# taishan1994/pytorch-distributed-NLP

Measured on NVIDIA H100. Metric: training samples/sec (seq_len=128), higher is better.
Workload: dtype bf16

## Files before the change

pytorch-distributed-nlp_b200/csrc/common.cuh:

```cuda
#pragma once
#include <cuda.h>
#include <cuda_bf16.h>
#include <cuda_runtime.h>
#include <stdint.h>
#include <cstdio>
#include "wgmma.cuh"

namespace b2 {

void set_error(const char* fmt, ...);
int32_t check_cuda(cudaError_t e, const char* what);
void count_launches(int n);
#define B2_CUDA(expr)                                                   \
  do {                                                                  \
    int32_t _s = ::b2::check_cuda((expr), #expr);                       \
    if (_s != 0) return _s;                                             \
  } while (0)
#define B2_REQUIRE(cond, ...)                                           \
  do {                                                                  \
    if (!(cond)) {                                                      \
      ::b2::set_error(__VA_ARGS__);                                     \
      return -2;                                                        \
    }                                                                   \
  } while (0)

int32_t get_tensor_map_2d(CUtensorMap* out, const void* base, uint64_t rows, uint64_t cols,
                          uint64_t pitch_bytes, uint32_t box_rows, uint32_t box_cols);

#ifdef __CUDACC__
template <typename... KArgs, typename... Args>
inline void launch_kernel(void (*kernel)(KArgs...), dim3 grid, dim3 block, size_t smem, cudaStream_t stream,
                          Args&&... args) {
  cudaLaunchConfig_t cfg = {};
  cfg.gridDim = grid;
  cfg.blockDim = block;
  cfg.dynamicSmemBytes = smem;
  cfg.stream = stream;
  cudaLaunchAttribute attr[1];
  attr[0].id = cudaLaunchAttributeProgrammaticStreamSerialization;
  attr[0].val.programmaticStreamSerializationAllowed = 1;
  cfg.attrs = attr;
  cfg.numAttrs = 1;
  (void)cudaLaunchKernelEx(&cfg, kernel, static_cast<KArgs>(args)...);
}
#define B2_LAUNCH(kernel, grid, block, smem, stream, ...) \
  ::b2::launch_kernel(kernel, dim3(grid), dim3(block), (size_t)(smem), (cudaStream_t)(stream), ##__VA_ARGS__)

__device__ __forceinline__ uint32_t smem_u32(const void* p) {
  return static_cast<uint32_t>(__cvta_generic_to_shared(p));
}
__device__ __forceinline__ uint8_t* smem_align_1024(uint8_t* smem_raw) {
  return smem_raw + ((1024u - (smem_u32(smem_raw) & 1023u)) & 1023u);
}
__device__ __forceinline__ uint32_t lane_id() { return threadIdx.x & 31; }

__device__ __forceinline__ float warp_sum(float v) {
#pragma unroll
  for (int o = 16; o > 0; o >>= 1) v += __shfl_xor_sync(0xffffffffu, v, o);
  return v;
}
__device__ __forceinline__ float warp_max(float v) {
#pragma unroll
  for (int o = 16; o > 0; o >>= 1) v = fmaxf(v, __shfl_xor_sync(0xffffffffu, v, o));
  return v;
}

__device__ __forceinline__ uint32_t pack_bf16(float lo, float hi) {
  __nv_bfloat162 t = __floats2bfloat162_rn(lo, hi);
  return *reinterpret_cast<uint32_t*>(&t);
}
__device__ __forceinline__ float bf16_lo(uint32_t v) { return __uint_as_float(v << 16); }
__device__ __forceinline__ float bf16_hi(uint32_t v) { return __uint_as_float(v & 0xffff0000u); }
__device__ __forceinline__ float bf16_round(float x) {
  return __bfloat162float(__float2bfloat16_rn(x));
}

__device__ __forceinline__ void gelu_hq(float x, float& hq, float& e) {
  float t;
  asm("ex2.approx.ftz.f32 %0, %1;" : "=f"(e) : "f"((x * x) * -0.72134752044448170f));
  asm("rcp.approx.ftz.f32 %0, %1;" : "=f"(t) : "f"(fmaf(fabsf(x), 0.23164189f, 1.0f)));
  float poly = fmaf(0.5307027145f, t, -0.7265760135f);
  poly = fmaf(poly, t, 0.7107068705f);
  poly = fmaf(poly, t, -0.142248368f);
  poly = fmaf(poly, t, 0.127414796f);
  hq = (poly * t) * e;
}
__device__ __forceinline__ float gelu_erf(float x) {
  float hq, e;
  gelu_hq(x, hq, e);
  return fmaf(-fabsf(x), hq, fmaxf(x, 0.f));
}
__device__ __forceinline__ float gelu_erf_grad(float x) {
  float hq, e;
  gelu_hq(x, hq, e);
  const float cdf = x >= 0.f ? 1.0f - hq : hq;
  return fmaf(x * 0.3989422804014327f, e, cdf);
}
__device__ __forceinline__ float ex2_approx(float x) {
  float y;
  asm("ex2.approx.ftz.f32 %0, %1;" : "=f"(y) : "f"(x));
  return y;
}
__device__ __forceinline__ uint32_t pack_bf16_round(float& lo, float& hi) {
  const uint32_t u = pack_bf16(lo, hi);
  lo = bf16_lo(u);
  hi = bf16_hi(u);
  return u;
}

struct Philox4 {
  uint32_t x, y, z, w;
};
__device__ __forceinline__ Philox4 philox4x32_10(uint32_t c0, uint32_t c1, uint32_t c2, uint32_t c3,
                                                 uint32_t k0, uint32_t k1) {
  const uint32_t M0 = 0xD2511F53u, M1 = 0xCD9E8D57u, W0 = 0x9E3779B9u, W1 = 0xBB67AE85u;
#pragma unroll
  for (int r = 0; r < 10; ++r) {
    const uint32_t hi0 = __umulhi(M0, c0), lo0 = M0 * c0;
    const uint32_t hi1 = __umulhi(M1, c2), lo1 = M1 * c2;
    const uint32_t n0 = hi1 ^ c1 ^ k0, n1 = lo1, n2 = hi0 ^ c3 ^ k1, n3 = lo0;
    c0 = n0; c1 = n1; c2 = n2; c3 = n3;
    k0 += W0; k1 += W1;
  }
  return Philox4{c0, c1, c2, c3};
}

struct DropCtx {
  uint32_t k0, k1, step, site, thresh;
  float scale;
};
__device__ __forceinline__ DropCtx make_drop_ctx(const unsigned long long* rng, uint32_t site, float p) {
  DropCtx d;
  unsigned long long seed = rng ? rng[0] : 0ull;
  unsigned long long step = rng ? rng[1] : 0ull;
  d.k0 = (uint32_t)seed; d.k1 = (uint32_t)(seed >> 32);
  d.step = (uint32_t)step; d.site = site;
  d.thresh = (uint32_t)(p * 65536.0f + 0.5f);
  d.scale = (p > 0.f) ? 1.0f / (1.0f - p) : 1.0f;
  return d;
}
__device__ __forceinline__ uint32_t dropout_keep8(const DropCtx& d, unsigned long long idx) {
  if (d.thresh == 0) return 0xffu;
  const unsigned long long g = idx >> 3;
  Philox4 r = philox4x32_10((uint32_t)g, (uint32_t)(g >> 32), d.site, d.step, d.k0, d.k1);
  uint32_t m = 0;
  m |= ((r.x & 0xffffu) >= d.thresh) << 0;
  m |= ((r.x >> 16) >= d.thresh) << 1;
  m |= ((r.y & 0xffffu) >= d.thresh) << 2;
  m |= ((r.y >> 16) >= d.thresh) << 3;
  m |= ((r.z & 0xffffu) >= d.thresh) << 4;
  m |= ((r.z >> 16) >= d.thresh) << 5;
  m |= ((r.w & 0xffffu) >= d.thresh) << 6;
  m |= ((r.w >> 16) >= d.thresh) << 7;
  return m;
}

__device__ __forceinline__ void mbar_init(uint64_t* bar, uint32_t count) {
  asm volatile("mbarrier.init.shared::cta.b64 [%0], %1;" ::"r"(smem_u32(bar)), "r"(count) : "memory");
}
__device__ __forceinline__ void fence_mbar_init() {
  asm volatile("fence.mbarrier_init.release.cluster;" ::: "memory");
}
__device__ __forceinline__ void mbar_expect_tx(uint64_t* bar, uint32_t bytes) {
  asm volatile("mbarrier.arrive.expect_tx.shared::cta.b64 _, [%0], %1;" ::"r"(smem_u32(bar)), "r"(bytes)
               : "memory");
}
__device__ __forceinline__ void mbar_arrive(uint64_t* bar) {
  asm volatile("mbarrier.arrive.shared::cta.b64 _, [%0];" ::"r"(smem_u32(bar)) : "memory");
}
__device__ __forceinline__ bool mbar_try_wait(uint64_t* bar, uint32_t parity) {
  uint32_t ok;
  asm volatile(
      "{\n\t.reg .pred p;\n\t"
      "mbarrier.try_wait.parity.shared::cta.b64 p, [%1], %2;\n\t"
      "selp.u32 %0, 1, 0, p;\n\t}"
      : "=r"(ok)
      : "r"(smem_u32(bar)), "r"(parity)
      : "memory");
  return ok != 0;
}
__device__ __forceinline__ void mbar_wait(uint64_t* bar, uint32_t parity) {
  uint32_t spins = 0;
  while (!mbar_try_wait(bar, parity)) {
    if (++spins > (1u << 24)) __trap();
  }
}

__device__ __forceinline__ void fence_proxy_async_smem() {
  asm volatile("fence.proxy.async.shared::cta;" ::: "memory");
}

__device__ __forceinline__ void tma_prefetch_desc(const CUtensorMap* m) {
  asm volatile("prefetch.tensormap [%0];" ::"l"(reinterpret_cast<uint64_t>(m)) : "memory");
}
__device__ __forceinline__ void tma_load_2d(void* smem_dst, const CUtensorMap* m, uint64_t* bar, int32_t c0,
                                            int32_t c1) {
  asm volatile(
      "cp.async.bulk.tensor.2d.shared::cluster.global.mbarrier::complete_tx::bytes [%0], [%1, {%3, %4}], [%2];"
      ::"r"(smem_u32(smem_dst)),
      "l"(reinterpret_cast<uint64_t>(m)), "r"(smem_u32(bar)), "r"(c0), "r"(c1)
      : "memory");
}
__device__ __forceinline__ void tma_store_2d(const CUtensorMap* m, const void* smem_src, int32_t c0, int32_t c1) {
  asm volatile("cp.async.bulk.tensor.2d.global.shared::cta.bulk_group [%0, {%2, %3}], [%1];" ::"l"(
                   reinterpret_cast<uint64_t>(m)),
               "r"(smem_u32(smem_src)), "r"(c0), "r"(c1)
               : "memory");
}
__device__ __forceinline__ void tma_store_commit_and_wait() {
  asm volatile("cp.async.bulk.commit_group;" ::: "memory");
  asm volatile("cp.async.bulk.wait_group 0;" ::: "memory");
}

__device__ __forceinline__ uint32_t cluster_ctarank() {
  uint32_t r;
  asm volatile("mov.u32 %0, %%cluster_ctarank;" : "=r"(r));
  return r;
}
__device__ __forceinline__ uint32_t mapa_u32(uint32_t smem_addr, uint32_t rank) {
  uint32_t r;
  asm volatile("mapa.shared::cluster.u32 %0, %1, %2;" : "=r"(r) : "r"(smem_addr), "r"(rank));
  return r;
}
__device__ __forceinline__ void st_cluster_f32x2(uint32_t cluster_addr, float a, float b) {
  asm volatile("st.shared::cluster.v2.f32 [%0], {%1, %2};" ::"r"(cluster_addr), "f"(a), "f"(b) : "memory");
}
__device__ __forceinline__ void cluster_sync_all() {
  asm volatile("barrier.cluster.arrive.release.aligned;\n\tbarrier.cluster.wait.acquire.aligned;" ::: "memory");
}
__device__ __forceinline__ void named_barrier_sync(uint32_t id, uint32_t count) {
  asm volatile("bar.sync %0, %1;" ::"r"(id), "r"(count) : "memory");
}

__device__ __forceinline__ uint64_t make_smem_desc(uint32_t saddr, uint32_t lbo_bytes, uint32_t sbo_bytes) {
  uint64_t d = 0;
  d |= (uint64_t)((saddr >> 4) & 0x3fffu);
  d |= (uint64_t)((lbo_bytes >> 4) & 0x3fffu) << 16;
  d |= (uint64_t)((sbo_bytes >> 4) & 0x3fffu) << 32;
  d |= (uint64_t)1 << 62;
  return d;
}

__device__ __forceinline__ void pdl_wait() { asm volatile("griddepcontrol.wait;" ::: "memory"); }
__device__ __forceinline__ void pdl_launch_dependents() { asm volatile("griddepcontrol.launch_dependents;" ::: "memory"); }

__device__ __forceinline__ uint4 ldg16(const void* p) { return __ldg(reinterpret_cast<const uint4*>(p)); }
__device__ __forceinline__ void stg16(void* p, uint4 v) { *reinterpret_cast<uint4*>(p) = v; }
#endif

}
```

pytorch-distributed-nlp_b200/csrc/gemm.cu:

```cuda
#include "common.cuh"
#include "gemm_epilogue.cuh"
#include "../../include/b2_ddp_bert.h"

namespace b2 {

constexpr int BM = 128;
constexpr int BK = 64;
constexpr int WGMMA_K = 16;
constexpr int kGemmThreads = (4 + kEpiWarps) * 32;

template <int BN>
struct GemmCfg {
  static constexpr int kABytes = BM * BK * 2;
  static constexpr int kBBytes = BN * BK * 2;
  static constexpr int kStageBytes = kABytes + kBBytes;
  static constexpr int kStages = (BN == 256) ? 4 : 6;
  static constexpr int kPipeBytes = kStages * kStageBytes;
  static constexpr int kAccLd = BN + 4;
  static constexpr int kSmemBytes = kPipeBytes + kEpiWarps * kEpiStageBytes + 1024  + 256 ;
  static_assert(BM * kAccLd * 4 <= kPipeBytes, "the accumulator tile lives in the drained operand ring");
};

template <int BN, bool A_MN, bool B_MN>
__device__ __forceinline__ void gemm_mainloop(uint8_t* smem, uint64_t* full_bar, uint64_t* empty_bar,
                                              const CUtensorMap* tmap_a, const CUtensorMap* tmap_b, int m0, int n0,
                                              int kb0, int kb1, int warp, int lane) {
  using Cfg = GemmCfg<BN>;
  if (warp == 0) {
    if (lane == 0) {
      int stage = 0; uint32_t phase = 0;
      for (int kb = kb0; kb < kb1; ++kb) {
        mbar_wait(&empty_bar[stage], phase ^ 1);
        mbar_expect_tx(&full_bar[stage], Cfg::kStageBytes);
        uint8_t* sa = smem + stage * Cfg::kStageBytes;
        uint8_t* sb = sa + Cfg::kABytes;
        const int k0 = kb * BK;
        if (!A_MN) {
          tma_load_2d(sa, tmap_a, &full_bar[stage], k0, m0);
        } else {
#pragma unroll
          for (int j = 0; j < BM / 64; ++j)
            tma_load_2d(sa + j * (BK * 128), tmap_a, &full_bar[stage], m0 + 64 * j, k0);
        }
        if (!B_MN) {
          tma_load_2d(sb, tmap_b, &full_bar[stage], k0, n0);
        } else {
#pragma unroll
          for (int j = 0; j < BN / 64; ++j)
            tma_load_2d(sb + j * (BK * 128), tmap_b, &full_bar[stage], n0 + 64 * j, k0);
        }
        if (++stage == Cfg::kStages) { stage = 0; phase ^= 1; }
      }
    }
  } else if (warp >= 4) {
    const int wg = (warp - 4) >> 2;
    constexpr uint32_t a_lbo = A_MN ? BK * 128 : 16, b_lbo = B_MN ? BK * 128 : 16;
    constexpr uint32_t a_kstep = A_MN ? WGMMA_K * 128 : WGMMA_K * 2;
    constexpr uint32_t b_kstep = B_MN ? WGMMA_K * 128 : WGMMA_K * 2;
    float acc[BN / 2];
#pragma unroll
    for (int i = 0; i < BN / 2; ++i) acc[i] = 0.f;
    int stage = 0, prev = -1; uint32_t phase = 0;
    for (int kb = kb0; kb < kb1; ++kb) {
      mbar_wait(&full_bar[stage], phase);
      const uint32_t sa = smem_u32(smem + stage * Cfg::kStageBytes) + wg * 8192;
      const uint32_t sb = smem_u32(smem + stage * Cfg::kStageBytes + Cfg::kABytes);
      wgmma_fence();
#pragma unroll
      for (int k = 0; k < BK / WGMMA_K; ++k)
        wgmma_bf16<BN, A_MN ? 1 : 0, B_MN ? 1 : 0>(acc, make_smem_desc(sa + k * a_kstep, a_lbo, 1024),
                                                     make_smem_desc(sb + k * b_kstep, b_lbo, 1024),
                                                     (kb > kb0 || k > 0) ? 1u : 0u);
      wgmma_commit();
      wgmma_wait<1>();
      if (prev >= 0 && lane == 0) mbar_arrive(&empty_bar[prev]);
      prev = stage;
      if (++stage == Cfg::kStages) { stage = 0; phase ^= 1; }
    }
    wgmma_wait<0>();
    wgmma_fence_regs(acc);
    if (prev >= 0 && lane == 0) mbar_arrive(&empty_bar[prev]);
    named_barrier_sync(1, kEpiWarps * 32);
    float* accs = reinterpret_cast<float*>(smem);
    const int r = wg * 64 + (warp & 3) * 16 + (lane >> 2);
    const int c = 2 * (lane & 3);
#pragma unroll
    for (int j = 0; j < BN / 8; ++j) {
      *reinterpret_cast<float2*>(accs + (size_t)r * Cfg::kAccLd + 8 * j + c) = make_float2(acc[4 * j], acc[4 * j + 1]);
      *reinterpret_cast<float2*>(accs + (size_t)(r + 8) * Cfg::kAccLd + 8 * j + c) =
          make_float2(acc[4 * j + 2], acc[4 * j + 3]);
    }
    named_barrier_sync(1, kEpiWarps * 32);
  }
}

template <int BN>
__device__ __forceinline__ void gemm_setup(uint64_t* full_bar, uint64_t* empty_bar) {
  if (threadIdx.x == 0) {
    for (int s = 0; s < GemmCfg<BN>::kStages; ++s) {
      mbar_init(&full_bar[s], 1);
      mbar_init(&empty_bar[s], kEpiWarps);
    }
    fence_mbar_init();
  }
  __syncthreads();
}

template <int BN, bool A_MN, bool B_MN>
__global__ void __launch_bounds__(kGemmThreads, 1)
gemm_bf16_kernel(const __grid_constant__ CUtensorMap tmap_a, const __grid_constant__ CUtensorMap tmap_b,
                 const GemmKernelParams p) {
  using Cfg = GemmCfg<BN>;
  extern __shared__ uint8_t smem_raw[];
  uint8_t* smem = smem_align_1024(smem_raw);
  uint8_t* epi_stage = smem + Cfg::kPipeBytes;
  uint64_t* full_bar = reinterpret_cast<uint64_t*>(epi_stage + kEpiWarps * kEpiStageBytes);
  uint64_t* empty_bar = full_bar + Cfg::kStages;
  const int warp = threadIdx.x >> 5;
  const int lane = threadIdx.x & 31;
  if (threadIdx.x == 0) {
    tma_prefetch_desc(&tmap_a);
    tma_prefetch_desc(&tmap_b);
  }
  gemm_setup<BN>(full_bar, empty_bar);
  pdl_wait();
  pdl_launch_dependents();

  const int tile = blockIdx.x / p.splits, split = blockIdx.x % p.splits;
  const int m0 = (tile / p.tiles_n) * BM, n0 = (tile % p.tiles_n) * BN;
  const int kb0 = split * p.kblocks_per_split;
  const int kb1 = min(kb0 + p.kblocks_per_split, p.kblocks_total);
  gemm_mainloop<BN, A_MN, B_MN>(smem, full_bar, empty_bar, &tmap_a, &tmap_b, m0, n0, kb0, kb1, warp, lane);
  if (warp >= 4) {
    const DropCtx drop = make_drop_ctx(p.rng, p.rng_site, p.dropout_p);
    epilogue_tile<BN>(p, drop, reinterpret_cast<const float*>(smem), Cfg::kAccLd, warp, lane, m0, n0, split,
                      epi_stage + (warp - 4) * kEpiStageBytes);
  }
}

constexpr int kMaxGroup = 4;
struct GroupedProblem {
  int M, N, tiles_n, tile_begin;
  __nv_bfloat16* D; long long ldd;
};
struct GroupedParams {
  int count, num_work, kblocks;
  GroupedProblem pr[kMaxGroup];
};

struct GroupedMaps {
  CUtensorMap a[kMaxGroup], b[kMaxGroup];
};
__device__ __forceinline__ int grouped_find(const GroupedParams& gp, int w) {
  int pi = 0;
#pragma unroll
  for (int i = 1; i < kMaxGroup; ++i)
    if (i < gp.count && w >= gp.pr[i].tile_begin) pi = i;
  return pi;
}

__global__ void __launch_bounds__(kGemmThreads, 1)
gemm_grouped_tn_kernel(const __grid_constant__ GroupedMaps maps, const GroupedParams gp) {
  constexpr int BN = 256;
  using Cfg = GemmCfg<BN>;
  extern __shared__ uint8_t smem_raw[];
  uint8_t* smem = smem_align_1024(smem_raw);
  uint8_t* epi_stage = smem + Cfg::kPipeBytes;
  uint64_t* full_bar = reinterpret_cast<uint64_t*>(epi_stage + kEpiWarps * kEpiStageBytes);
  uint64_t* empty_bar = full_bar + Cfg::kStages;
  const int warp = threadIdx.x >> 5;
  const int lane = threadIdx.x & 31;
  const int pi = grouped_find(gp, blockIdx.x);
  if (threadIdx.x == 0) {
    tma_prefetch_desc(&maps.a[pi]);
    tma_prefetch_desc(&maps.b[pi]);
  }
  gemm_setup<BN>(full_bar, empty_bar);
  pdl_wait();
  pdl_launch_dependents();

  const GroupedProblem& pr = gp.pr[pi];
  const int lt = blockIdx.x - pr.tile_begin;
  const int m0 = (lt / pr.tiles_n) * BM;
  const int n0 = (lt % pr.tiles_n) * BN;
  gemm_mainloop<BN, true, true>(smem, full_bar, empty_bar, &maps.a[pi], &maps.b[pi], m0, n0, 0, gp.kblocks, warp,
                                lane);
  if (warp < 4) return;
  uint8_t* stage = epi_stage + (warp - 4) * kEpiStageBytes;
  GemmKernelParams q;
  q.splits = 1; q.epilogue = B2_EPI_NONE; q.bias = nullptr; q.aux_in = nullptr; q.aux_out = nullptr;
  q.partial = nullptr; q.dropout_p = 0.f; q.rng = nullptr; q.rng_site = 0; q.timing = nullptr; q.colsum = nullptr;
  q.ld_aux_in = 0; q.ld_aux_out = 0; q.K = 0; q.tiles_m = 0; q.kblocks_per_split = 0; q.kblocks_total = 0;
  q.M = pr.M; q.N = pr.N; q.tiles_n = pr.tiles_n; q.D = pr.D; q.ldd = pr.ldd;
  DropCtx drop;
  drop.k0 = 0; drop.k1 = 0; drop.step = 0; drop.site = 0; drop.thresh = 0; drop.scale = 1.f;
  epilogue_tile<BN>(q, drop, reinterpret_cast<const float*>(smem), Cfg::kAccLd, warp, lane, m0, n0, 0, stage);
}

__global__ void splitk_reduce_kernel(const float* __restrict__ partial, __nv_bfloat16* __restrict__ D,
                                     long long ldd, int M, int N, int splits) {
  pdl_wait();
  pdl_launch_dependents();
  const long long idx = (long long)blockIdx.x * blockDim.x + threadIdx.x;
  const long long total = (long long)M * N / 4;
  if (idx >= total) return;
  const long long e = idx * 4;
  const int m = (int)(e / N), n = (int)(e % N);
  float4 acc = make_float4(0.f, 0.f, 0.f, 0.f);
  for (int s = 0; s < splits; ++s) {
    const float4 v = *reinterpret_cast<const float4*>(partial + (size_t)s * M * N + e);
    acc.x += v.x; acc.y += v.y; acc.z += v.z; acc.w += v.w;
  }
  uint2 o;
  o.x = pack_bf16(acc.x, acc.y);
  o.y = pack_bf16(acc.z, acc.w);
  *reinterpret_cast<uint2*>(D + (size_t)m * ldd + n) = o;
}

static int g_num_sms = 0;
static int num_sms() {
  if (g_num_sms == 0) {
    int dev = 0;
    cudaGetDevice(&dev);
    cudaDeviceGetAttribute(&g_num_sms, cudaDevAttrMultiProcessorCount, dev);
    if (g_num_sms <= 0) g_num_sms = 132;
  }
  return g_num_sms;
}

static void fill_params(GemmKernelParams& p, const b2_gemm_args_t& a, int tile_m, int bn, int splits) {
  p.M = (int)a.M; p.N = (int)a.N; p.K = (int)a.K;
  p.tiles_m = (p.M + tile_m - 1) / tile_m;
  p.tiles_n = (p.N + bn - 1) / bn;
  p.kblocks_total = (p.K + BK - 1) / BK;
  p.splits = splits;
  p.kblocks_per_split = (p.kblocks_total + splits - 1) / splits;
  p.epilogue = (splits > 1 && a.epilogue != B2_EPI_ACCUM_F32) ? B2_EPI_PARTIAL_F32 : a.epilogue;
  p.D = (__nv_bfloat16*)a.D; p.ldd = a.ldd;
  p.bias = (const __nv_bfloat16*)a.bias;
  p.aux_in = (const __nv_bfloat16*)a.aux_in; p.ld_aux_in = a.ld_aux_in;
  p.aux_out = (__nv_bfloat16*)a.aux_out; p.ld_aux_out = a.ld_aux_out;
  p.partial = (float*)a.workspace;
  p.dropout_p = a.dropout_p; p.rng = (const unsigned long long*)a.rng_state; p.rng_site = a.rng_site;
  p.timing = (long long*)a.debug_timing;
  p.colsum = a.colsum_out;
}

static int32_t launch_splitk_reduce(const b2_gemm_args_t& a, int splits, cudaStream_t stream) {
  const long long total = (long long)a.M * a.N / 4;
  B2_LAUNCH(splitk_reduce_kernel, (unsigned)((total + 255) / 256), 256, 0, stream, 
      (const float*)a.workspace, (__nv_bfloat16*)a.D, a.ldd, (int)a.M, (int)a.N, splits);
  B2_CUDA(cudaGetLastError());
  count_launches(1);
  return 0;
}

template <int BN, bool A_MN, bool B_MN>
static int32_t launch_gemm(const b2_gemm_args_t& a, int splits, cudaStream_t stream) {
  using Cfg = GemmCfg<BN>;
  CUtensorMap ta, tb;
  int32_t st;
  if (!A_MN) st = get_tensor_map_2d(&ta, a.A, (uint64_t)a.M, (uint64_t)a.K, (uint64_t)a.lda * 2, BM, 64);
  else       st = get_tensor_map_2d(&ta, a.A, (uint64_t)a.K, (uint64_t)a.M, (uint64_t)a.lda * 2, BK, 64);
  if (st) return st;
  if (!B_MN) st = get_tensor_map_2d(&tb, a.B, (uint64_t)a.N, (uint64_t)a.K, (uint64_t)a.ldb * 2, BN, 64);
  else       st = get_tensor_map_2d(&tb, a.B, (uint64_t)a.K, (uint64_t)a.N, (uint64_t)a.ldb * 2, BK, 64);
  if (st) return st;
  GemmKernelParams p;
  fill_params(p, a, BM, BN, splits);
  auto kern = gemm_bf16_kernel<BN, A_MN, B_MN>;
  static bool attr_set = false;
  if (!attr_set) {
    B2_CUDA(cudaFuncSetAttribute(kern, cudaFuncAttributeMaxDynamicSharedMemorySize, Cfg::kSmemBytes));
    attr_set = true;
  }
  const int work = p.tiles_m * p.tiles_n * p.splits;
  B2_LAUNCH(kern, work, kGemmThreads, Cfg::kSmemBytes, stream, ta, tb, p);
  B2_CUDA(cudaGetLastError());
  count_launches(1);
  if (splits > 1 && a.epilogue != B2_EPI_ACCUM_F32) return launch_splitk_reduce(a, splits, stream);
  return 0;
}

struct Choice { int bn, splits; };
static Choice choose_config(const b2_gemm_args_t& a) {
  const int sms = num_sms();
  const int kblocks = (int)((a.K + BK - 1) / BK);
  const bool accum = a.epilogue == B2_EPI_ACCUM_F32;
  const bool can_split = accum || ((a.epilogue == B2_EPI_NONE) && a.workspace != nullptr && a.bias == nullptr);
  double best = 1e30;
  Choice c{128, 1};
  const double l2_bytes_per_cycle = 3000.0;
  const int bns[2] = {256, 128};
  for (int bi = 0; bi < 2; ++bi) {
    const int bn = bns[bi];
    if (a.N % bn != 0 && bn != 128) continue;
    const int tiles = (int)((a.M + BM - 1) / BM) * (int)((a.N + bn - 1) / bn);
    const int max_s = can_split ? 8 : 1;
    for (int s = 1; s <= max_s; s = accum ? s + 1 : s * 2) {
      if (s > 1 && (kblocks / s < 8)) break;
      if (s > 1 && !accum && (size_t)s * a.M * a.N * 4 > (size_t)a.workspace_bytes) break;
      const int work = tiles * s;
      const int rounds = (work + sms - 1) / sms;
      const int busy_sms = work < sms ? work : sms;
      const double mma_cycles = 128.0 * bn * 64 / 2048.0;
      const double bytes_per_sm = (128 + bn) * 128.0;
      const double feed_cycles = bytes_per_sm * busy_sms / l2_bytes_per_cycle;
      const double kb_cycles = mma_cycles > feed_cycles ? mma_cycles : feed_cycles;
      double t = rounds * ((double)((kblocks + s - 1) / s) * kb_cycles + 2500.0 );
      if (s > 1 && !accum) t += 1500.0 + (double)s * a.M * a.N * 8 / 3000.0;
      if (s > 1 && accum) t += (double)(s - 1) * a.M * a.N * 4 / 3000.0;
      if (t < best) { best = t; c = Choice{bn, s}; }
    }
  }
  return c;
}

}

using namespace b2;

extern "C" int32_t b2_gemm_bf16(const b2_gemm_args_t* a, void* stream_) {
  cudaStream_t stream = (cudaStream_t)stream_;
  B2_REQUIRE(a != nullptr, "b2_gemm_bf16: null args");
  B2_REQUIRE(a->M > 0 && a->N > 0 && a->K > 0, "b2_gemm_bf16: empty problem M=%lld N=%lld K=%lld",
             (long long)a->M, (long long)a->N, (long long)a->K);
  B2_REQUIRE(a->A && a->B && a->D, "b2_gemm_bf16: null operand pointer");
  B2_REQUIRE(a->N % 64 == 0, "b2_gemm_bf16: N=%lld must be a multiple of 64", (long long)a->N);
  B2_REQUIRE(a->K % 8 == 0 && a->lda % 8 == 0 && a->ldb % 8 == 0 && a->ldd % 8 == 0,
             "b2_gemm_bf16: K and leading dimensions must be multiples of 8 elements (16 B)");
  B2_REQUIRE(((uintptr_t)a->A % 16 == 0) && ((uintptr_t)a->B % 16 == 0) && ((uintptr_t)a->D % 16 == 0),
             "b2_gemm_bf16: operands must be 16-byte aligned");
  B2_REQUIRE(a->epilogue >= B2_EPI_NONE && a->epilogue <= B2_EPI_ACCUM_F32, "b2_gemm_bf16: bad epilogue %d",
             a->epilogue);
  if (a->epilogue == B2_EPI_BIAS || a->epilogue == B2_EPI_BIAS_GELU || a->epilogue == B2_EPI_BIAS_DROPOUT_RESIDUAL)
    B2_REQUIRE(a->bias != nullptr, "b2_gemm_bf16: epilogue %d needs a bias", a->epilogue);
  if (a->epilogue == B2_EPI_BIAS_DROPOUT_RESIDUAL || a->epilogue == B2_EPI_RESIDUAL ||
      a->epilogue == B2_EPI_GELU_BWD || a->epilogue == B2_EPI_RESIDUAL_F32)
    B2_REQUIRE(a->aux_in != nullptr && a->ld_aux_in % 8 == 0, "b2_gemm_bf16: epilogue %d needs aux_in",
               a->epilogue);
  if (a->epilogue == B2_EPI_BIAS_GELU)
    B2_REQUIRE(a->aux_out != nullptr && a->ld_aux_out % 8 == 0, "b2_gemm_bf16: BIAS_GELU needs aux_out");
  if (a->epilogue == B2_EPI_BIAS_DROPOUT_RESIDUAL && a->dropout_p > 0.f)
    B2_REQUIRE(a->rng_state != nullptr, "b2_gemm_bf16: dropout needs rng_state");
  B2_REQUIRE(a->dropout_p >= 0.f && a->dropout_p < 1.f, "b2_gemm_bf16: dropout_p out of range");

  Choice c = choose_config(*a);
  if (a->force_bn == 128 || a->force_bn == 256) {
    B2_REQUIRE(a->N % a->force_bn == 0 || a->force_bn == 128, "b2_gemm_bf16: force_bn does not divide N");
    c.bn = a->force_bn;
  }
  if (a->force_splits >= 1) {
    B2_REQUIRE(a->force_splits == 1 ||
                   a->epilogue == B2_EPI_ACCUM_F32 ||
                   (a->epilogue == B2_EPI_NONE && a->workspace &&
                    (size_t)a->force_splits * a->M * a->N * 4 <= (size_t)a->workspace_bytes),
               "b2_gemm_bf16: split-K needs EPI_ACCUM_F32, or EPI_NONE and a large enough workspace");
    c.splits = a->force_splits;
  }
  const bool a_mn = a->a_major == B2_MAJOR_MN, b_mn = a->b_major == B2_MAJOR_MN;
  B2_REQUIRE(!(a_mn && !b_mn), "b2_gemm_bf16: layout TT (A MN-major, B K-major) is not on the path");

#define B2_DISPATCH(BN_)                                                          \
  if (c.bn == BN_) {                                                              \
    if (!a_mn && !b_mn) return launch_gemm<BN_, false, false>(*a, c.splits, stream); \
    if (!a_mn && b_mn) return launch_gemm<BN_, false, true>(*a, c.splits, stream);   \
    return launch_gemm<BN_, true, true>(*a, c.splits, stream);                       \
  }
  B2_DISPATCH(128)
  B2_DISPATCH(256)
#undef B2_DISPATCH
  set_error("b2_gemm_bf16: no kernel for BN=%d", c.bn);
  return -2;
}

extern "C" int32_t b2_gemm_bf16_grouped(const b2_gemm_args_t* args, int32_t count, void* stream_) {
  cudaStream_t stream = (cudaStream_t)stream_;
  B2_REQUIRE(args != nullptr && count >= 1, "b2_gemm_bf16_grouped: no problems");
  bool groupable = count <= kMaxGroup;
  for (int i = 0; i < count && groupable; ++i) {
    const b2_gemm_args_t& a = args[i];
    groupable = a.a_major == B2_MAJOR_MN && a.b_major == B2_MAJOR_MN && a.epilogue == B2_EPI_NONE &&
                a.bias == nullptr && a.colsum_out == nullptr && a.N % 256 == 0 && a.K == args[0].K && a.M > 0 &&
                a.K > 0 && a.A && a.B && a.D && a.K % 8 == 0 && a.lda % 8 == 0 && a.ldb % 8 == 0 &&
                a.ldd % 8 == 0 && ((uintptr_t)a.A % 16 == 0) && ((uintptr_t)a.B % 16 == 0) &&
                ((uintptr_t)a.D % 16 == 0) && a.force_splits <= 1 &&
                (a.force_bn == 0 || a.force_bn == 256);
  }
  if (!groupable) {
    for (int i = 0; i < count; ++i) {
      const int32_t st = b2_gemm_bf16(&args[i], stream_);
      if (st) return st;
    }
    return 0;
  }
  GroupedMaps maps;
  GroupedParams gp;
  gp.count = count;
  gp.kblocks = (int)((args[0].K + BK - 1) / BK);
  int work = 0;
  for (int i = 0; i < count; ++i) {
    const b2_gemm_args_t& a = args[i];
    int32_t st = get_tensor_map_2d(&maps.a[i], a.A, (uint64_t)a.K, (uint64_t)a.M, (uint64_t)a.lda * 2, BK, 64);
    if (st) return st;
    st = get_tensor_map_2d(&maps.b[i], a.B, (uint64_t)a.K, (uint64_t)a.N, (uint64_t)a.ldb * 2, BK, 64);
    if (st) return st;
    GroupedProblem& g = gp.pr[i];
    g.M = (int)a.M; g.N = (int)a.N; g.tiles_n = (int)(a.N / 256); g.tile_begin = work;
    g.D = (__nv_bfloat16*)a.D; g.ldd = a.ldd;
    work += (int)((a.M + BM - 1) / BM) * g.tiles_n;
  }
  for (int i = count; i < kMaxGroup; ++i) { gp.pr[i] = gp.pr[0]; gp.pr[i].tile_begin = 0x7fffffff; maps.a[i] = maps.a[0]; maps.b[i] = maps.b[0]; }
  gp.num_work = work;
  static bool attr_set = false;
  if (!attr_set) {
    B2_CUDA(cudaFuncSetAttribute(gemm_grouped_tn_kernel, cudaFuncAttributeMaxDynamicSharedMemorySize,
                                 GemmCfg<256>::kSmemBytes));
    attr_set = true;
  }
  B2_LAUNCH(gemm_grouped_tn_kernel, work, kGemmThreads, GemmCfg<256>::kSmemBytes, stream, maps, gp);
  B2_CUDA(cudaGetLastError());
  count_launches(1);
  return 0;
}
```

pytorch-distributed-nlp_b200/csrc/gemm_epilogue.cuh:

```cuda
#pragma once
#include "common.cuh"
#include "../../include/b2_ddp_bert.h"

namespace b2 {

struct GemmKernelParams {
  int M, N, K;
  int tiles_m, tiles_n, splits, kblocks_per_split, kblocks_total;
  int epilogue;
  __nv_bfloat16* D; long long ldd;
  const __nv_bfloat16* bias;
  const __nv_bfloat16* aux_in; long long ld_aux_in;
  __nv_bfloat16* aux_out; long long ld_aux_out;
  float* partial;
  float dropout_p; const unsigned long long* rng; unsigned rng_site;
  long long* timing;
  float* colsum;
};

constexpr int kEpiStageBytes = 32 * 128;

#ifdef __CUDACC__
template <int CH>
__device__ __forceinline__ uint4* stage_ptr(uint8_t* stage, int row, int chunk) {
  if (CH == 8) return reinterpret_cast<uint4*>(stage + row * 128 + ((chunk ^ (row & 7)) << 4));
  return reinterpret_cast<uint4*>(stage + (row >> 1) * 128 + (((((row & 1) << 2) | chunk) ^ ((row >> 1) & 7)) << 4));
}
template <int CH>
__device__ __forceinline__ void tile_s2g(uint8_t* stage, uint8_t* g, long long pitch, int lane, int rows_valid) {
  constexpr int RPS = 32 / CH;
#pragma unroll
  for (int k = 0; k < CH; ++k) {
    const int r = RPS * k + lane / CH, c = lane % CH;
    const uint4 v = *stage_ptr<CH>(stage, r, c);
    if (r < rows_valid) *reinterpret_cast<uint4*>(g + (size_t)r * pitch + c * 16) = v;
  }
}
__device__ __forceinline__ void tile_s2g_red_f32(uint8_t* stage, uint8_t* g, long long pitch, int lane,
                                                 int rows_valid) {
#pragma unroll
  for (int k = 0; k < 8; ++k) {
    const int r = 4 * k + (lane >> 3), c = lane & 7;
    const uint4 v = *stage_ptr<8>(stage, r, c);
    if (r < rows_valid)
      asm volatile("red.global.add.v4.f32 [%0], {%1, %2, %3, %4};" ::"l"(g + (size_t)r * pitch + c * 16),
                   "f"(__uint_as_float(v.x)), "f"(__uint_as_float(v.y)), "f"(__uint_as_float(v.z)),
                   "f"(__uint_as_float(v.w))
                   : "memory");
  }
}
template <int CH>
__device__ __forceinline__ void tile_g2s_async(uint8_t* stage, const uint8_t* g, long long pitch, int lane,
                                               int rows_valid) {
  constexpr int RPS = 32 / CH;
#pragma unroll
  for (int k = 0; k < CH; ++k) {
    const int r = RPS * k + lane / CH, c = lane % CH;
    uint4* dst = stage_ptr<CH>(stage, r, c);
    if (r < rows_valid) {
      asm volatile("cp.async.cg.shared.global [%0], [%1], 16;" ::"r"(smem_u32(dst)), "l"(g + (size_t)r * pitch + c * 16)
                   : "memory");
    } else {
      *dst = make_uint4(0u, 0u, 0u, 0u);
    }
  }
  asm volatile("cp.async.commit_group;" ::: "memory");
}
__device__ __forceinline__ void tile_async_wait() { asm volatile("cp.async.wait_group 0;" ::: "memory"); }

__device__ __forceinline__ void acc_ld32(const float* a, uint32_t (&v)[32]) {
#pragma unroll
  for (int k = 0; k < 8; ++k) {
    const uint4 t = *reinterpret_cast<const uint4*>(a + 4 * k);
    v[4 * k] = t.x; v[4 * k + 1] = t.y; v[4 * k + 2] = t.z; v[4 * k + 3] = t.w;
  }
}

template <int CH>
__device__ __forceinline__ void row_write32(uint8_t* stage, int lane, int c0, const float (&f)[32]) {
#pragma unroll
  for (int c = 0; c < 4; ++c) {
    uint4 o;
    o.x = pack_bf16(f[8 * c + 0], f[8 * c + 1]); o.y = pack_bf16(f[8 * c + 2], f[8 * c + 3]);
    o.z = pack_bf16(f[8 * c + 4], f[8 * c + 5]); o.w = pack_bf16(f[8 * c + 6], f[8 * c + 7]);
    *stage_ptr<CH>(stage, lane, c0 + c) = o;
  }
}
template <int CH>
__device__ __forceinline__ void row_read32(uint8_t* stage, int lane, int c0, float (&r)[32]) {
#pragma unroll
  for (int c = 0; c < 4; ++c) {
    const uint4 t = *stage_ptr<CH>(stage, lane, c0 + c);
    r[8 * c + 0] = bf16_lo(t.x); r[8 * c + 1] = bf16_hi(t.x); r[8 * c + 2] = bf16_lo(t.y); r[8 * c + 3] = bf16_hi(t.y);
    r[8 * c + 4] = bf16_lo(t.z); r[8 * c + 5] = bf16_hi(t.z); r[8 * c + 6] = bf16_lo(t.w); r[8 * c + 7] = bf16_hi(t.w);
  }
}

constexpr int kEpiWarps = 8;
template <int BN>
__device__ __forceinline__ void epilogue_tile(const GemmKernelParams& p, const DropCtx& drop, const float* acc,
                                              int acc_ld, int warp, int lane, int m_base, int n0, int split,
                                              uint8_t* stage) {
  static_assert(BN == 128 || BN == 256, "tile widths on the path");
  constexpr int kColsPerWarp = BN / 2;
  constexpr int WT = 64;
  constexpr int CH = WT / 8;
  const int quarter = warp & 3;
  const int cgrp = (warp - 4) >> 2;
  const int row0 = m_base + quarter * 32;
  const int rows_valid = p.M - row0;
  const int m = row0 + lane;
  const int nw = n0 + cgrp * kColsPerWarp;
  const float* arow = acc + (size_t)(quarter * 32 + lane) * acc_ld + cgrp * kColsPerWarp;

  if (p.epilogue == B2_EPI_PARTIAL_F32 || p.epilogue == B2_EPI_RESIDUAL_F32 || p.epilogue == B2_EPI_ACCUM_F32) {
    const bool accum = p.epilogue == B2_EPI_ACCUM_F32;
    const bool no_aux = p.epilogue != B2_EPI_RESIDUAL_F32;
    const bool to_ws = p.epilogue == B2_EPI_PARTIAL_F32;
    float* dst_base = to_ws ? p.partial + (size_t)split * p.M * p.N : reinterpret_cast<float*>(p.D);
    const long long dst_ld = to_ws ? (long long)p.N : p.ldd;
    auto prefetch = [&](int c) {
      const int n = nw + c * 32;
      if (!no_aux && n < p.N && rows_valid > 0)
        tile_g2s_async<8>(stage, reinterpret_cast<const uint8_t*>(reinterpret_cast<const float*>(p.aux_in) +
                                                                 (size_t)row0 * p.ld_aux_in + n),
                          p.ld_aux_in * 4, lane, rows_valid);
    };
    prefetch(0);
#pragma unroll 1
    for (int c = 0; c < kColsPerWarp / 32; ++c) {
      const int n = nw + c * 32;
      uint32_t v[32];
      acc_ld32(arow + c * 32, v);
      if (n < p.N && rows_valid > 0) {
        if (!no_aux) {
          if (c > 0) prefetch(c);
          tile_async_wait();
          __syncwarp();
#pragma unroll
          for (int k = 0; k < 8; ++k) {
            const uint4 t = *stage_ptr<8>(stage, lane, k);
            v[4 * k + 0] = __float_as_uint(__uint_as_float(v[4 * k + 0]) + __uint_as_float(t.x));
            v[4 * k + 1] = __float_as_uint(__uint_as_float(v[4 * k + 1]) + __uint_as_float(t.y));
            v[4 * k + 2] = __float_as_uint(__uint_as_float(v[4 * k + 2]) + __uint_as_float(t.z));
            v[4 * k + 3] = __float_as_uint(__uint_as_float(v[4 * k + 3]) + __uint_as_float(t.w));
          }
          __syncwarp();
        }
#pragma unroll
        for (int k = 0; k < 8; ++k)
          *stage_ptr<8>(stage, lane, k) = make_uint4(v[4 * k], v[4 * k + 1], v[4 * k + 2], v[4 * k + 3]);
        __syncwarp();
        uint8_t* gdst = reinterpret_cast<uint8_t*>(dst_base + (size_t)row0 * dst_ld + n);
        if (accum) tile_s2g_red_f32(stage, gdst, dst_ld * 4, lane, rows_valid);
        else       tile_s2g<8>(stage, gdst, dst_ld * 4, lane, rows_valid);
      }
      __syncwarp();
    }
    return;
  }

  const bool has_aux = p.epilogue == B2_EPI_BIAS_DROPOUT_RESIDUAL || p.epilogue == B2_EPI_RESIDUAL ||
                       p.epilogue == B2_EPI_GELU_BWD;
  auto prefetch = [&](int t) {
    const int n = nw + t * WT;
    if (has_aux && n < p.N && rows_valid > 0)
      tile_g2s_async<CH>(stage, reinterpret_cast<const uint8_t*>(p.aux_in + (size_t)row0 * p.ld_aux_in + n),
                         p.ld_aux_in * 2, lane, rows_valid);
  };
  prefetch(0);
#pragma unroll 1
  for (int t = 0; t < kColsPerWarp / WT; ++t) {
    const int n = nw + t * WT;
    const bool active = n < p.N && rows_valid > 0;
    if (has_aux && active) {
      if (t > 0) prefetch(t);
      tile_async_wait();
      __syncwarp();
    }
#pragma unroll 1
    for (int h = 0; h < WT / 32; ++h) {
      float f[32];
      {
        uint32_t v[32];
        acc_ld32(arow + t * WT + h * 32, v);
#pragma unroll
        for (int j = 0; j < 32; ++j) f[j] = __uint_as_float(v[j]);
      }
      if (!active) continue;
      const int nh = n + h * 32;
      if (p.bias != nullptr) {
#pragma unroll
        for (int j = 0; j < 32; j += 8) {
          const uint4 b = ldg16(p.bias + nh + j);
          f[j + 0] += bf16_lo(b.x); f[j + 1] += bf16_hi(b.x); f[j + 2] += bf16_lo(b.y); f[j + 3] += bf16_hi(b.y);
          f[j + 4] += bf16_lo(b.z); f[j + 5] += bf16_hi(b.z); f[j + 6] += bf16_lo(b.w); f[j + 7] += bf16_hi(b.w);
        }
      }
      if (has_aux) {
        float r[32];
        row_read32<CH>(stage, lane, 4 * h, r);
        if (p.epilogue == B2_EPI_BIAS_DROPOUT_RESIDUAL) {
#pragma unroll
          for (int j = 0; j < 32; j += 8) {
            const uint32_t keep = dropout_keep8(drop, (unsigned long long)m * p.N + nh + j);
#pragma unroll
            for (int i = 0; i < 8; ++i) f[j + i] = (((keep >> i) & 1u) ? f[j + i] * drop.scale : 0.f) + r[j + i];
          }
        } else if (p.epilogue == B2_EPI_RESIDUAL) {
#pragma unroll
          for (int j = 0; j < 32; ++j) f[j] += r[j];
        } else {
#pragma unroll
          for (int j = 0; j < 32; ++j) f[j] *= gelu_erf_grad(r[j]);
        }
      }
      row_write32<CH>(stage, lane, 4 * h, f);
    }
    if (active) {
      __syncwarp();
      if (p.epilogue == B2_EPI_BIAS_GELU) {
        tile_s2g<CH>(stage, reinterpret_cast<uint8_t*>(p.aux_out + (size_t)row0 * p.ld_aux_out + n), p.ld_aux_out * 2,
                     lane, rows_valid);
        __syncwarp();
#pragma unroll 1
        for (int h = 0; h < WT / 32; ++h) {
          float f[32];
          row_read32<CH>(stage, lane, 4 * h, f);
#pragma unroll
          for (int j = 0; j < 32; ++j) f[j] = gelu_erf(f[j]);
          row_write32<CH>(stage, lane, 4 * h, f);
        }
        __syncwarp();
      }
      if (p.colsum != nullptr) {
        float s0 = 0.f, s1 = 0.f;
        const int nr = rows_valid < 32 ? rows_valid : 32;
        if (WT == 64 || lane < 16) {
          for (int r = 0; r < nr; ++r) {
            const uint32_t w = *reinterpret_cast<const uint32_t*>(
                reinterpret_cast<const uint8_t*>(stage_ptr<CH>(stage, r, lane >> 2)) + (lane & 3) * 4);
            s0 += bf16_lo(w);
            s1 += bf16_hi(w);
          }
          atomicAdd(p.colsum + n + 2 * lane, s0);
          atomicAdd(p.colsum + n + 2 * lane + 1, s1);
        }
      }
      tile_s2g<CH>(stage, reinterpret_cast<uint8_t*>(p.D + (size_t)row0 * p.ldd + n), p.ldd * 2, lane, rows_valid);
    }
    __syncwarp();
  }
}
#endif

}
```

Before: 4515.

## Add warp-specialized persistent GEMM kernel overlapping epilogue with next tile mainloop

Adds a persistent GEMM kernel with a producer warp, two MMA warpgroups and dedicated epilogue warps. Each CTA loops over tiles, staging accumulators in a swizzled shared-memory buffer guarded by mbarriers so the epilogue of one tile overlaps the mainloop of the next. Register budgets are rebalanced across roles with setmaxnreg. It is selected when tile count is at least twice the SM count with no split-K. It also adds optional globaltimer instrumentation, which adds a branch and needs a timing field in the params.

```diff
diff --git a/pytorch-distributed-nlp_b200/csrc/common.cuh b/pytorch-distributed-nlp_b200/csrc/common.cuh
--- a/pytorch-distributed-nlp_b200/csrc/common.cuh
+++ b/pytorch-distributed-nlp_b200/csrc/common.cuh
@@ -53,6 +53,16 @@
   return smem_raw + ((1024u - (smem_u32(smem_raw) & 1023u)) & 1023u);
 }
 __device__ __forceinline__ uint32_t lane_id() { return threadIdx.x & 31; }
+__device__ __forceinline__ long long globaltimer_ns() {
+  long long t;
+  asm volatile("mov.u64 %0, %%globaltimer;" : "=l"(t));
+  return t;
+}
+__device__ __forceinline__ uint32_t sm_id() {
+  uint32_t r;
+  asm volatile("mov.u32 %0, %%smid;" : "=r"(r));
+  return r;
+}
 
 __device__ __forceinline__ float warp_sum(float v) {
 #pragma unroll
diff --git a/pytorch-distributed-nlp_b200/csrc/gemm.cu b/pytorch-distributed-nlp_b200/csrc/gemm.cu
--- a/pytorch-distributed-nlp_b200/csrc/gemm.cu
+++ b/pytorch-distributed-nlp_b200/csrc/gemm.cu
@@ -118,6 +118,8 @@
   uint64_t* empty_bar = full_bar + Cfg::kStages;
   const int warp = threadIdx.x >> 5;
   const int lane = threadIdx.x & 31;
+  long long* t_start = reinterpret_cast<long long*>(empty_bar + Cfg::kStages);
+  if (p.timing && threadIdx.x == 128) *t_start = globaltimer_ns();
   if (threadIdx.x == 0) {
     tma_prefetch_desc(&tmap_a);
     tma_prefetch_desc(&tmap_b);
@@ -132,9 +134,165 @@
   const int kb1 = min(kb0 + p.kblocks_per_split, p.kblocks_total);
   gemm_mainloop<BN, A_MN, B_MN>(smem, full_bar, empty_bar, &tmap_a, &tmap_b, m0, n0, kb0, kb1, warp, lane);
   if (warp >= 4) {
+    if (p.timing && threadIdx.x == 128) stamp_mainloop(p.timing, blockIdx.x, *t_start);
     const DropCtx drop = make_drop_ctx(p.rng, p.rng_site, p.dropout_p);
     epilogue_tile<BN>(p, drop, reinterpret_cast<const float*>(smem), Cfg::kAccLd, warp, lane, m0, n0, split,
                       epi_stage + (warp - 4) * kEpiStageBytes);
+    if (p.timing) {
+      named_barrier_sync(1, kEpiWarps * 32);
+      if (threadIdx.x == 128) stamp_epilogue(p.timing, blockIdx.x);
+    }
+  }
+}
+
+constexpr int kPersistThreads = (4 + 8 + kEpiWarps) * 32;
+constexpr uint32_t kRegsProducer = 24, kRegsMma = 104, kRegsEpi = 120;
+struct PersistCfg {
+  static constexpr int kStages = 4;
+  static constexpr int kStageBytes = GemmCfg<128>::kStageBytes;
+  static constexpr int kPipeBytes = kStages * kStageBytes;
+  static constexpr int kAccBytes = BM * 128 * 4;
+  static constexpr int kSmemBytes = kPipeBytes + kAccBytes + kEpiWarps * kEpiStageBytes + 1024  +
+                                    256 ;
+  static_assert(kSmemBytes <= 232448, "one CTA per SM: 227 KB of shared memory");
+};
+template <uint32_t R>
+__device__ __forceinline__ void setmaxnreg_inc() { asm volatile("setmaxnreg.inc.sync.aligned.u32 %0;" ::"n"(R)); }
+template <uint32_t R>
+__device__ __forceinline__ void setmaxnreg_dec() { asm volatile("setmaxnreg.dec.sync.aligned.u32 %0;" ::"n"(R)); }
+__device__ __forceinline__ void st_shared_f32x2(uint32_t addr, float a, float b) {
+  asm volatile("st.shared.v2.f32 [%0], {%1, %2};" ::"r"(addr), "f"(a), "f"(b) : "memory");
+}
+
+template <bool A_MN, bool B_MN>
+__global__ void __launch_bounds__(kPersistThreads, 1)
+gemm_persistent_kernel(const __grid_constant__ CUtensorMap tmap_a, const __grid_constant__ CUtensorMap tmap_b,
+                       const __grid_constant__ GemmKernelParams p) {
+  constexpr int BN = 128;
+  using Cfg = PersistCfg;
+  extern __shared__ uint8_t smem_raw[];
+  uint8_t* smem = smem_align_1024(smem_raw);
+  float* accs = reinterpret_cast<float*>(smem + Cfg::kPipeBytes);
+  uint8_t* epi_stage = smem + Cfg::kPipeBytes + Cfg::kAccBytes;
+  uint64_t* full_bar = reinterpret_cast<uint64_t*>(epi_stage + kEpiWarps * kEpiStageBytes);
+  uint64_t* empty_bar = full_bar + Cfg::kStages;
+  uint64_t* acc_full = empty_bar + Cfg::kStages;
+  uint64_t* acc_empty = acc_full + 1;
+  long long* t_start = reinterpret_cast<long long*>(acc_empty + 1);
+  const int warp = threadIdx.x >> 5;
+  const int lane = threadIdx.x & 31;
+  if (threadIdx.x == 0) {
+    tma_prefetch_desc(&tmap_a);
+    tma_prefetch_desc(&tmap_b);
+    for (int s = 0; s < Cfg::kStages; ++s) {
+      mbar_init(&full_bar[s], 1);
+      mbar_init(&empty_bar[s], 8);
+    }
+    mbar_init(acc_full, 256);
+    mbar_init(acc_empty, kEpiWarps * 32);
+    fence_mbar_init();
+  }
+  __syncthreads();
+  pdl_wait();
+  const int nwork = p.tiles_m * p.tiles_n;
+  long long* timing = p.timing;
+
+  if (warp < 4) {
+    setmaxnreg_dec<kRegsProducer>();
+    if (warp == 0 && lane == 0) {
+      int stage = 0; uint32_t phase = 0;
+      for (int w = blockIdx.x; w < nwork; w += gridDim.x) {
+        const int m0 = (w % p.tiles_m) * BM, n0 = (w / p.tiles_m) * BN;
+        for (int kb = 0; kb < p.kblocks_total; ++kb) {
+          mbar_wait(&empty_bar[stage], phase ^ 1);
+          mbar_expect_tx(&full_bar[stage], Cfg::kStageBytes);
+          uint8_t* sa = smem + stage * Cfg::kStageBytes;
+          uint8_t* sb = sa + GemmCfg<BN>::kABytes;
+          const int k0 = kb * BK;
+          if (!A_MN) {
+            tma_load_2d(sa, &tmap_a, &full_bar[stage], k0, m0);
+          } else {
+#pragma unroll
+            for (int j = 0; j < BM / 64; ++j)
+              tma_load_2d(sa + j * (BK * 128), &tmap_a, &full_bar[stage], m0 + 64 * j, k0);
+          }
+          if (!B_MN) {
+            tma_load_2d(sb, &tmap_b, &full_bar[stage], k0, n0);
+          } else {
+#pragma unroll
+            for (int j = 0; j < BN / 64; ++j)
+              tma_load_2d(sb + j * (BK * 128), &tmap_b, &full_bar[stage], n0 + 64 * j, k0);
+          }
+          if (++stage == Cfg::kStages) { stage = 0; phase ^= 1; }
+        }
+      }
+    }
+  } else if (warp < 12) {
+    setmaxnreg_inc<kRegsMma>();
+    const int wg = (warp - 4) >> 2;
+    constexpr uint32_t a_lbo = A_MN ? BK * 128 : 16, b_lbo = B_MN ? BK * 128 : 16;
+    constexpr uint32_t a_kstep = A_MN ? WGMMA_K * 128 : WGMMA_K * 2;
+    constexpr uint32_t b_kstep = B_MN ? WGMMA_K * 128 : WGMMA_K * 2;
+    const int r = wg * 64 + (warp & 3) * 16 + (lane >> 2);
+    const uint32_t acc_row = smem_u32(accs) + r * 512;
+    const int c = 2 * (lane & 3);
+    int stage = 0; uint32_t phase = 0, acc_phase = 0;
+    for (int w = blockIdx.x; w < nwork; w += gridDim.x) {
+      if (timing != nullptr && threadIdx.x == 128) *t_start = globaltimer_ns();
+      float acc[BN / 2];
+#pragma unroll
+      for (int i = 0; i < BN / 2; ++i) acc[i] = 0.f;
+      int prev = -1;
+      for (int kb = 0; kb < p.kblocks_total; ++kb) {
+        mbar_wait(&full_bar[stage], phase);
+        const uint32_t sa = smem_u32(smem + stage * Cfg::kStageBytes) + wg * 8192;
+        const uint32_t sb = smem_u32(smem + stage * Cfg::kStageBytes + GemmCfg<BN>::kABytes);
+        wgmma_fence();
+#pragma unroll
+        for (int k = 0; k < BK / WGMMA_K; ++k)
+          wgmma_bf16<BN, A_MN ? 1 : 0, B_MN ? 1 : 0>(acc, make_smem_desc(sa + k * a_kstep, a_lbo, 1024),
+                                                       make_smem_desc(sb + k * b_kstep, b_lbo, 1024),
+                                                       (kb > 0 || k > 0) ? 1u : 0u);
+        wgmma_commit();
+        wgmma_wait<1>();
+        if (prev >= 0 && lane == 0) mbar_arrive(&empty_bar[prev]);
+        prev = stage;
+        if (++stage == Cfg::kStages) { stage = 0; phase ^= 1; }
+      }
+      wgmma_wait<0>();
+      wgmma_fence_regs(acc);
+      if (prev >= 0 && lane == 0) mbar_arrive(&empty_bar[prev]);
+      if (w + (int)gridDim.x >= nwork) pdl_launch_dependents();
+      if (timing != nullptr && threadIdx.x == 128) stamp_mainloop(timing, w, *t_start);
+      mbar_wait(acc_empty, acc_phase ^ 1);
+#pragma unroll
+      for (int j = 0; j < BN / 8; ++j) {
+        const int ch = 2 * j + (c >> 2);
+        const uint32_t a = acc_row + (((ch & ~7) | ((ch ^ r) & 7)) << 4) + (c & 3) * 4;
+        st_shared_f32x2(a, acc[4 * j], acc[4 * j + 1]);
+        st_shared_f32x2(a + 8 * 512, acc[4 * j + 2], acc[4 * j + 3]);
+      }
+      mbar_arrive(acc_full);
+      acc_phase ^= 1;
+    }
+  } else {
+    setmaxnreg_inc<kRegsEpi>();
+    const DropCtx drop = make_drop_ctx(p.rng, p.rng_site, p.dropout_p);
+    uint8_t* stage = epi_stage + (warp - 12) * kEpiStageBytes;
+    uint32_t acc_phase = 0;
+#pragma unroll 1
+    for (int w = blockIdx.x; w < nwork; w += gridDim.x) {
+      const int m0 = (w % p.tiles_m) * BM, n0 = (w / p.tiles_m) * BN;
+      mbar_wait(acc_full, acc_phase);
+      if (w + (int)gridDim.x >= nwork) pdl_launch_dependents();
+      epilogue_tile<BN>(p, drop, accs, 128, warp - 8, lane, m0, n0, 0, stage, true);
+      mbar_arrive(acc_empty);
+      acc_phase ^= 1;
+      if (timing != nullptr) {
+        named_barrier_sync(1, kEpiWarps * 32);
+        if (warp == 12 && lane == 0) stamp_epilogue(timing, w);
+      }
+    }
   }
 }
 
@@ -279,6 +437,31 @@
   B2_CUDA(cudaGetLastError());
   count_launches(1);
   if (splits > 1 && a.epilogue != B2_EPI_ACCUM_F32) return launch_splitk_reduce(a, splits, stream);
+  return 0;
+}
+
+template <bool A_MN, bool B_MN>
+static int32_t launch_persistent(const b2_gemm_args_t& a, cudaStream_t stream) {
+  CUtensorMap ta, tb;
+  int32_t st;
+  if (!A_MN) st = get_tensor_map_2d(&ta, a.A, (uint64_t)a.M, (uint64_t)a.K, (uint64_t)a.lda * 2, BM, 64);
+  else       st = get_tensor_map_2d(&ta, a.A, (uint64_t)a.K, (uint64_t)a.M, (uint64_t)a.lda * 2, BK, 64);
+  if (st) return st;
+  if (!B_MN) st = get_tensor_map_2d(&tb, a.B, (uint64_t)a.N, (uint64_t)a.K, (uint64_t)a.ldb * 2, 128, 64);
+  else       st = get_tensor_map_2d(&tb, a.B, (uint64_t)a.K, (uint64_t)a.N, (uint64_t)a.ldb * 2, BK, 64);
+  if (st) return st;
+  GemmKernelParams p;
+  fill_params(p, a, BM, 128, 1);
+  auto kern = gemm_persistent_kernel<A_MN, B_MN>;
+  static bool attr_set = false;
+  if (!attr_set) {
+    B2_CUDA(cudaFuncSetAttribute(kern, cudaFuncAttributeMaxDynamicSharedMemorySize, PersistCfg::kSmemBytes));
+    attr_set = true;
+  }
+  B2_LAUNCH(kern, std::min(p.tiles_m * p.tiles_n, num_sms()), kPersistThreads, PersistCfg::kSmemBytes, stream, ta, tb,
+            p);
+  B2_CUDA(cudaGetLastError());
+  count_launches(1);
   return 0;
 }
 
@@ -316,6 +499,11 @@
   return c;
 }
 
+static bool persistent_pays(const b2_gemm_args_t& a) {
+  const long long tiles = ((a.M + BM - 1) / BM) * ((a.N + 127) / 128);
+  return tiles >= 2LL * num_sms();
+}
+
 }
 
 using namespace b2;
@@ -360,6 +548,14 @@
   }
   const bool a_mn = a->a_major == B2_MAJOR_MN, b_mn = a->b_major == B2_MAJOR_MN;
   B2_REQUIRE(!(a_mn && !b_mn), "b2_gemm_bf16: layout TT (A MN-major, B K-major) is not on the path");
+  bool persistent = a->force_kernel == 2 ? (c.bn == 128 && c.splits == 1)
+                  : a->force_kernel == 1 ? false
+                  : (c.splits == 1 && a->force_bn != 256 && persistent_pays(*a));
+  if (persistent) {
+    if (!a_mn && !b_mn) return launch_persistent<false, false>(*a, stream);
+    if (!a_mn && b_mn) return launch_persistent<false, true>(*a, stream);
+    return launch_persistent<true, true>(*a, stream);
+  }
 
 #define B2_DISPATCH(BN_)                                                          \
   if (c.bn == BN_) {                                                              \
diff --git a/pytorch-distributed-nlp_b200/csrc/gemm_epilogue.cuh b/pytorch-distributed-nlp_b200/csrc/gemm_epilogue.cuh
--- a/pytorch-distributed-nlp_b200/csrc/gemm_epilogue.cuh
+++ b/pytorch-distributed-nlp_b200/csrc/gemm_epilogue.cuh
@@ -21,6 +21,17 @@
 constexpr int kEpiStageBytes = 32 * 128;
 
 #ifdef __CUDACC__
+__device__ __forceinline__ void stamp_mainloop(long long* timing, int w, long long t_start) {
+  timing[4 * (size_t)w] = t_start;
+  timing[4 * (size_t)w + 1] = globaltimer_ns();
+}
+__device__ __forceinline__ void stamp_epilogue(long long* timing, int w) {
+  timing[4 * (size_t)w + 2] = globaltimer_ns();
+  atomicAdd(reinterpret_cast<unsigned long long*>(timing + 4 * (size_t)w + 3), (1ull << 32) | sm_id());
+}
+#endif
+
+#ifdef __CUDACC__
 template <int CH>
 __device__ __forceinline__ uint4* stage_ptr(uint8_t* stage, int row, int chunk) {
   if (CH == 8) return reinterpret_cast<uint4*>(stage + row * 128 + ((chunk ^ (row & 7)) << 4));
@@ -68,10 +79,10 @@
 }
 __device__ __forceinline__ void tile_async_wait() { asm volatile("cp.async.wait_group 0;" ::: "memory"); }
 
-__device__ __forceinline__ void acc_ld32(const float* a, uint32_t (&v)[32]) {
+__device__ __forceinline__ void acc_ld32(const float* a, int swz, uint32_t (&v)[32]) {
 #pragma unroll
   for (int k = 0; k < 8; ++k) {
-    const uint4 t = *reinterpret_cast<const uint4*>(a + 4 * k);
+    const uint4 t = *reinterpret_cast<const uint4*>(a + 4 * (k ^ swz));
     v[4 * k] = t.x; v[4 * k + 1] = t.y; v[4 * k + 2] = t.z; v[4 * k + 3] = t.w;
   }
 }
@@ -100,7 +111,7 @@
 template <int BN>
 __device__ __forceinline__ void epilogue_tile(const GemmKernelParams& p, const DropCtx& drop, const float* acc,
                                               int acc_ld, int warp, int lane, int m_base, int n0, int split,
-                                              uint8_t* stage) {
+                                              uint8_t* stage, bool swizzled = false) {
   static_assert(BN == 128 || BN == 256, "tile widths on the path");
   constexpr int kColsPerWarp = BN / 2;
   constexpr int WT = 64;
@@ -112,6 +123,7 @@
   const int m = row0 + lane;
   const int nw = n0 + cgrp * kColsPerWarp;
   const float* arow = acc + (size_t)(quarter * 32 + lane) * acc_ld + cgrp * kColsPerWarp;
+  const int swz = swizzled ? (lane & 7) : 0;
 
   if (p.epilogue == B2_EPI_PARTIAL_F32 || p.epilogue == B2_EPI_RESIDUAL_F32 || p.epilogue == B2_EPI_ACCUM_F32) {
     const bool accum = p.epilogue == B2_EPI_ACCUM_F32;
@@ -131,7 +143,7 @@
     for (int c = 0; c < kColsPerWarp / 32; ++c) {
       const int n = nw + c * 32;
       uint32_t v[32];
-      acc_ld32(arow + c * 32, v);
+      acc_ld32(arow + c * 32, swz, v);
       if (n < p.N && rows_valid > 0) {
         if (!no_aux) {
           if (c > 0) prefetch(c);
@@ -183,7 +195,7 @@
       float f[32];
       {
         uint32_t v[32];
-        acc_ld32(arow + t * WT + h * 32, v);
+        acc_ld32(arow + t * WT + h * 32, swz, v);
 #pragma unroll
         for (int j = 0; j < 32; ++j) f[j] = __uint_as_float(v[j]);
       }
```

After: 4678 (median of 6 runs). 3.6% higher.
